# SharperJBCA/COMAPreduce

Hardware: AMD Instinct MI355X
Metric: TOD samples x channels / s (L1 -> L2 reduction) (higher is better)
Workload: dtype f32 in, f64 accumulate

## Files before the change

### comapreduce_amd/_native.py

```python
import ctypes
import os
import threading

_HERE = os.path.dirname(os.path.abspath(__file__))
LIB_PATH = os.environ.get('COMAP_HIP_LIB') or os.path.join(_HERE, '_lib', 'libcomap_hip.so')

_lib = None
_lock = threading.Lock()
_ctx = {}

c_int, c_int32, c_int64, c_double, c_void_p = ctypes.c_int, ctypes.c_int32, ctypes.c_int64, ctypes.c_double, ctypes.c_void_p
P_double = ctypes.POINTER(ctypes.c_double)
P_int32 = ctypes.POINTER(ctypes.c_int32)
P_int64 = ctypes.POINTER(ctypes.c_int64)


class ObsDesc(ctypes.Structure):
    _fields_ = [('n_feeds', c_int32), ('n_bands', c_int32), ('n_channels', c_int32),
                ('n_scans', c_int32), ('n_samples', c_int64), ('tod', c_void_p), ('el', c_void_p),
                ('n_units', c_int32), ('units_host', P_int32)]


_SIGS = {
    'comap_ctx_create': (c_int, [c_int, ctypes.POINTER(c_void_p)]),
    'comap_ctx_destroy': (c_int, [c_void_p]),
    'comap_last_error': (ctypes.c_char_p, [c_void_p]),
    'comap_set_stream': (c_int, [c_void_p, c_void_p]),
    'comap_synchronize': (c_int, [c_void_p]),
    'comap_version': (ctypes.c_char_p, []),
    'comap_host_alloc': (c_int, [ctypes.c_size_t, ctypes.POINTER(c_void_p)]),
    'comap_host_free': (None, [c_void_p]),
    'comap_cache_trim': (c_int, []),
    'comap_cache_bytes': (c_int, [P_int64, P_int64, P_int64]),
    'comap_medfilt_f64': (c_int, [c_void_p, P_double, c_int64, c_int32]),
    'comap_medfilt_batch_f64': (c_int, [c_void_p, P_double, P_int64, c_int32, c_int32, c_int32, P_double]),
    'comap_bin_values_f64': (c_int, [c_void_p, P_double, c_int64, P_int64, P_double, P_int64, c_int64]),
    'comap_l1_plan_create': (c_int, [c_void_p, ctypes.POINTER(ObsDesc), ctypes.POINTER(c_void_p)]),
    'comap_l1_plan_destroy': (c_int, [c_void_p]),
    'comap_l1_vane': (c_int, [c_void_p, c_int64, c_int64, P_int32, P_int64, P_int32, P_int64, c_double,
                              c_void_p, c_void_p]),
    'comap_l1_prefetch': (c_int, [c_void_p]),
    'comap_l1_atmosphere': (c_int, [c_void_p, P_int32, c_int32, c_void_p]),
    'comap_l1_average': (c_int, [c_void_p, c_void_p, c_void_p, c_void_p, c_int32, c_void_p, c_void_p, c_void_p]),
    'comap_l1_debug_fetch': (c_int, [c_void_p, c_int32, P_double, c_int64]),
    'comap_l1_channel_bin': (c_int, [c_void_p, c_int32, c_void_p, c_void_p, c_void_p, c_void_p, c_void_p]),
    'comap_l1_profile': (c_int, [c_void_p, c_int32]),
    'comap_l1_profile_collect': (c_int, [c_void_p, P_double, P_int64, c_int32]),
    'comap_spikes': (c_int, [c_void_p, c_void_p, c_int32, c_int64, P_int64, c_int32, c_int32, c_int32, c_double,
                             c_void_p]),
    'comap_power_spectra': (c_int, [c_void_p, c_void_p, c_int32, c_int64, P_int64, c_int32, c_void_p, c_int32,
                                    P_int64, c_void_p]),
    'comap_synth_tod': (c_int, [c_void_p, c_int32, c_int32, c_int64, ctypes.c_uint64, c_void_p, c_void_p, c_void_p,
                                c_void_p, c_void_p]),
    'comap_destripe_create': (c_int, [c_void_p, c_void_p, c_void_p, c_void_p, c_int64, c_int32, c_int64,
                                      ctypes.POINTER(c_void_p)]),
    'comap_destripe_dist_bin': (c_int, [c_void_p, c_void_p, c_void_p, c_void_p]),
    'comap_destripe_dist_parts': (c_int32, []),
    'comap_destripe_dist_project_parts': (c_int, [c_void_p, c_void_p, c_void_p, c_void_p, c_void_p, c_void_p,
                                                  c_void_p]),
    'comap_destripe_dist_update_fused': (c_int, [c_void_p, c_void_p, c_void_p, c_void_p, c_void_p, c_void_p,
                                                 c_void_p, c_void_p, c_void_p]),
    'comap_destripe_dist_direction_fused': (c_int, [c_void_p, c_void_p, c_void_p, c_void_p, c_void_p, c_void_p]),
    'comap_destripe_create_bands': (c_int, [c_void_p, c_void_p, c_void_p, c_void_p, c_void_p, c_int64, c_int32,
                                            c_int64, c_int32, ctypes.POINTER(c_void_p)]),
    'comap_destripe_create_keyed': (c_int, [c_void_p, c_void_p, c_void_p, c_void_p, c_void_p, c_void_p, c_int64,
                                            c_int64, c_int32, c_int64, c_int32, ctypes.POINTER(c_void_p)]),
    'comap_offset_centroid_keys': (c_int, [c_void_p, c_void_p, c_int64, c_int32, c_int64, c_int64, c_void_p, c_int64,
                                           c_void_p]),
    'comap_destripe_destroy': (c_int, [c_void_p]),
    'comap_destripe_n_offsets': (c_int64, [c_void_p]),
    'comap_destripe_n_bands': (c_int32, [c_void_p]),
    'comap_destripe_offsets_natural': (c_int, [c_void_p, c_void_p, c_void_p]),
    'comap_destripe_nnz': (c_int, [c_void_p, P_int64, P_int64]),
    'comap_destripe_entry_bytes': (ctypes.c_int32, [c_void_p]),
    'comap_destripe_sell_entries': (c_int64, [c_void_p]),
    'comap_destripe_local_maps': (c_int, [c_void_p, c_void_p, c_void_p, c_void_p]),
    'comap_destripe_bin': (c_int, [c_void_p, c_void_p, c_int32, c_void_p]),
    'comap_destripe_project': (c_int, [c_void_p, c_void_p, c_void_p, c_void_p, c_void_p, c_void_p]),
    'comap_destripe_dot': (c_int, [c_void_p, c_void_p, c_void_p, c_void_p]),
    'comap_destripe_cg_update': (c_int, [c_void_p, c_void_p, c_void_p, c_void_p, c_void_p, c_void_p, c_void_p,
                                         c_void_p]),
    'comap_destripe_cg_direction': (c_int, [c_void_p, c_void_p, c_void_p, c_void_p, c_void_p]),
    'comap_destripe_div_map': (c_int, [c_void_p, c_void_p, c_void_p, c_void_p]),
    'comap_relabel_pixels': (c_int, [c_void_p, c_void_p, c_int64, c_void_p, c_int64, c_int64, c_void_p]),
    'comap_relabel_pixels_tiled': (c_int, [c_void_p, c_void_p, c_int64, c_int64, c_int64, c_int32, c_void_p]),
    'comap_destripe_solve': (c_int, [c_void_p, c_double, c_int32, c_void_p, c_void_p, c_void_p, c_void_p,
                                     c_void_p, P_int32]),
    'comap_destripe_ground_create': (c_int, [c_void_p, c_void_p, c_void_p, c_void_p, c_void_p, c_void_p, c_int64,
                                             ctypes.POINTER(c_void_p)]),
    'comap_destripe_ground_destroy': (c_int, [c_void_p]),
    'comap_destripe_ground_n_groups': (c_int64, [c_void_p]),
    'comap_destripe_ground_nnz': (c_int, [c_void_p, P_int64, P_int64]),
    'comap_destripe_ground_stats': (c_int, [c_void_p, c_void_p, c_void_p]),
    'comap_destripe_ground_fold': (c_int, [c_void_p, c_void_p, c_void_p, c_void_p]),
    'comap_destripe_ground_bin': (c_int, [c_void_p, c_void_p, c_void_p]),
    'comap_destripe_ground_project': (c_int, [c_void_p, c_void_p, c_void_p, c_void_p, c_void_p, c_void_p, c_void_p]),
    'comap_destripe_ground_rhs': (c_int, [c_void_p, c_void_p, c_void_p, c_void_p, c_void_p]),
    'comap_destripe_ground_tail_dot': (c_int, [c_void_p, c_void_p, c_void_p, c_void_p]),
    'comap_destripe_ground_tail_update': (c_int, [c_void_p, c_void_p, c_void_p, c_void_p, c_void_p, c_void_p, c_void_p,
                                                  c_void_p]),
    'comap_destripe_ground_tail_direction': (c_int, [c_void_p, c_void_p, c_void_p, c_void_p, c_void_p]),
    'comap_destripe_ground_wrapped': (c_int, [c_void_p, c_void_p]),
    'comap_destripe_ground_solve': (c_int, [c_void_p, c_double, c_int32, c_void_p, c_void_p, c_void_p, c_void_p,
                                            c_void_p, P_int32]),
    'comap_destripe_ground_dist_bin': (c_int, [c_void_p, c_void_p, c_void_p, c_void_p]),
    'comap_destripe_ground_dist_project': (c_int, [c_void_p, c_void_p, c_void_p, c_void_p, c_void_p, c_void_p,
                                                   c_void_p]),
    'comap_destripe_ground_dist_update': (c_int, [c_void_p, c_void_p, c_void_p, c_void_p, c_void_p, c_void_p,
                                                  c_void_p]),
    'comap_destripe_ground_dist_direction': (c_int, [c_void_p, c_void_p, c_void_p, c_void_p, c_void_p]),
    'comap_destripe_prior_create': (c_int, [c_void_p, c_void_p, c_int64, c_void_p, c_int32, ctypes.POINTER(c_void_p)]),
    'comap_destripe_prior_destroy': (c_int, [c_void_p]),
    'comap_destripe_prior_tile': (c_int32, []),
    'comap_destripe_prior_apply': (c_int, [c_void_p, c_void_p, c_void_p, c_int32]),
    'comap_destripe_prior_apply_dot': (c_int, [c_void_p, c_void_p, c_void_p, c_int32, c_void_p]),
    'comap_destripe_prior_solve': (c_int, [c_void_p, c_double, c_int32, c_void_p, c_void_p, c_void_p, c_void_p,
                                           c_void_p, P_int32]),
    'comap_destripe_mask_view': (c_int, [c_void_p, c_void_p, c_void_p, c_void_p, c_void_p, ctypes.POINTER(c_void_p)]),
    'comap_destripe_solve_view': (c_int, [c_void_p, c_double, c_int32, c_void_p, c_void_p, c_void_p, c_void_p,
                                          c_void_p, P_int32]),
    'comap_destripe_split_maps': (c_int, [c_void_p, c_void_p, c_void_p, c_void_p, c_void_p, c_void_p, c_void_p, c_int32,
                                          c_int64, c_int32, c_int64, c_int32, c_void_p, c_void_p, c_void_p, c_void_p]),
    'comap_destripe_split_div': (c_int, [c_void_p, c_void_p, c_void_p, c_void_p, c_int64, c_void_p, c_void_p]),
# ... 149 lines not shown
```

### comapreduce_amd/csrc/l1_kernels.hip

```cpp
#include "comap_internal.h"

#include <algorithm>
#include <cfloat>
#include <cmath>
#include <cstdlib>
#include <cstring>
#include <type_traits>
#include <utility>

using namespace comap;

#ifndef COMAP_GROUPS
#define COMAP_GROUPS 0
#endif
constexpr int kGroupsAutoMin = 3;

typedef float f32x4u __attribute__((ext_vector_type(4), aligned(4)));
__device__ __forceinline__ f32x4u ld4(const float *p)
{
    return __builtin_nontemporal_load(reinterpret_cast<const f32x4u *>(p));
}

__device__ __forceinline__ double wave_sum(double v)
{
// ... 218 lines not shown
        const int f = units[4 * u], t0 = units[4 * u + 2], n = units[4 * u + 3];
        const int t = blockIdx.x * blockDim.x + threadIdx.x;
        if (t >= n) continue;
        const float *p = tod + (int64_t)(f * kBands + b) * kChannels * T + t0 + t;
        bool ok = true;
        for (int c = 10; c < 1014; ++c)
            if (atmos_channel(c) && !isfinite(p[(int64_t)c * T])) ok = false;
        valid[voff[pr] + t] = ok;
    }
}

__global__ void __launch_bounds__(256) k_masked_fit_sums(const float *__restrict__ tod, const double *__restrict__ A,
                                                         const int32_t *__restrict__ units,
                                                         const int32_t *__restrict__ pairs, int64_t T,
                                                         const int64_t *__restrict__ voff,
                                                         const uint8_t *__restrict__ valid, int64_t UC,
                                                         double *__restrict__ fs, double *__restrict__ ub,
                                                         const int32_t *__restrict__ list,
                                                         const int32_t *__restrict__ count)
{
    const int np = *count;
    for (int li = blockIdx.y; li < np; li += gridDim.y) {
    const int pr = list[li];
    const int u = pairs[2 * pr], b = pairs[2 * pr + 1];
    const int f = units[4 * u], t0 = units[4 * u + 2], n = units[4 * u + 3];
    const int wid = threadIdx.x >> 6, lane = threadIdx.x & 63;
    const int c = blockIdx.x * 4 + wid;
    const float *p = tod + ((int64_t)(f * kBands + b) * kChannels + c) * T + t0;
    const double *a = A + (int64_t)f * T + t0;
    const uint8_t *v = valid + voff[pr];
    double s0 = 0, s1 = 0, cn = 0, sa = 0, saa = 0;
    for (int t = lane; t < n; t += 64) {
        if (!v[t]) continue;
        const double x = p[t], at = a[t];
        s0 += x;
        s1 = fma(at, x, s1);
        cn += 1.0;
        sa += at;
        saa = fma(at, at, saa);
    }
    s0 = wave_sum(s0); s1 = wave_sum(s1);
    cn = wave_sum(cn); sa = wave_sum(sa); saa = wave_sum(saa);
    if (lane == 0) {
        const int64_t i = (int64_t)u * kBC + b * kChannels + c;
        fs[i] = s0;
        fs[UC + i] = s1;
        if (c == 0) {
            double *o = ub + 4 * ((int64_t)u * kBands + b);
            o[0] = cn; o[1] = sa; o[2] = saa;
        }
    }
    }
}

__global__ void __launch_bounds__(256) k_pair_flags(const int32_t *__restrict__ rowbad, int npairs,
                                                    int32_t *__restrict__ flag)
{
    const int lane = threadIdx.x & 63;
    const int pr = blockIdx.x * 4 + (threadIdx.x >> 6);
    if (pr >= npairs) return;
    const int u = pr / kBands, b = pr % kBands;
    const int32_t *rb = rowbad + (int64_t)u * kBC + b * kChannels;
    bool any = false;
    for (int c = lane; c < kChannels; c += 64) any |= atmos_channel(c) && rb[c] > 0;
    any = __ballot(any) != 0ull;
    if (lane == 0) flag[pr] = any ? 1 : 0;
}

__global__ void k_pair_list(const int32_t *__restrict__ flag, int npairs, int32_t *__restrict__ list,
                            int32_t *__restrict__ count)
{
    const int lane = threadIdx.x & 63;
    int base = 0;
    for (int i0 = 0; i0 < npairs; i0 += 64) {
        const int i = i0 + lane;
        const bool f = i < npairs && flag[i];
        const unsigned long long m = __ballot(f);
        if (f) list[base + __popcll(m & ((1ull << lane) - 1ull))] = i;
        base += __popcll(m);
    }
    if (lane == 0) *count = base;
}

__global__ void k_ub_from_units(const double *__restrict__ us, int U, double *__restrict__ ub)
{
    const int i = blockIdx.x * blockDim.x + threadIdx.x;
    if (i >= U * kBands) return;
    const double *q = us + 8 * (int64_t)(i / kBands);
    ub[4 * (int64_t)i] = q[0];
    ub[4 * (int64_t)i + 1] = q[1];
    ub[4 * (int64_t)i + 2] = q[2];
}

__global__ void __launch_bounds__(256) k_fill_rows(float *__restrict__ tod, const int64_t *__restrict__ rows,
                                                   const float *__restrict__ med, int nrows, int64_t *__restrict__ pos,
                                                   int64_t cap, int64_t *__restrict__ npos)
{
    const int r = blockIdx.y;
    if (r >= nrows) return;
    const int64_t off = rows[2 * r];
    float *p = tod + off;
    const int64_t n = rows[2 * r + 1];
    const float m = med[r];
    for (int64_t i = blockIdx.x * (int64_t)blockDim.x + threadIdx.x; i < n; i += (int64_t)gridDim.x * blockDim.x)
        if (isnan(p[i])) {
            const unsigned long long k = atomicAdd(reinterpret_cast<unsigned long long *>(npos), 1ull);
            if ((int64_t)k < cap) {
                pos[k] = off + i;
                p[i] = m;
            }
        }
}

__global__ void k_restore_nan(float *__restrict__ tod, const int64_t *__restrict__ pos, const int64_t *__restrict__ npos,
                              int64_t cap)
{
    const int64_t n = min(*npos, cap);
    for (int64_t i = blockIdx.x * (int64_t)blockDim.x + threadIdx.x; i < n; i += (int64_t)gridDim.x * blockDim.x)
        tod[pos[i]] = __int_as_float(0x7fc00000);
}

__global__ void k_fit_from_median(const int32_t *__restrict__ units, const int32_t *__restrict__ ulist, int nu,
                                  const float *__restrict__ med, int F, double *__restrict__ fit)
{
    const int64_t i = blockIdx.x * (int64_t)blockDim.x + threadIdx.x;
    if (i >= (int64_t)nu * kBC) return;
    const int k = (int)(i / kBC), bc = (int)(i % kBC);
    const int u = ulist[k];
    const int f = units[4 * u], s = units[4 * u + 1];
    const int b = bc / kChannels, c = bc % kChannels;
    double *o = fit + (((int64_t)s * F + f) * kBands + b) * 2 * kChannels;
    o[c] = (double)med[i];
    o[kChannels + c] = 0.0;
}

__global__ void k_atmos_fit(const int32_t *__restrict__ units, const double *__restrict__ ubs,
                            const double *__restrict__ fs, int64_t UC, int F, int U,
                            double *__restrict__ fit, const double *__restrict__ fs_sel = nullptr,
                            const int32_t *__restrict__ sel = nullptr)
{
    const int64_t i = blockIdx.x * (int64_t)blockDim.x + threadIdx.x;
    if (i >= (int64_t)U * kBC) return;
    const int u = (int)(i / kBC);
    const int bc = (int)(i % kBC);
    const int b = bc / kChannels, c = bc % kChannels;
    const int f = units[4 * u], s = units[4 * u + 1];
    const double *q = ubs + 4 * ((int64_t)u * kBands + b);
    const double n = q[0], sa = q[1], saa = q[2];
    double o = NAN, a = NAN;
    if (atmos_channel(c) && n >= 100.0) {
        const double *src = (sel && sel[(int64_t)u * kBands + b]) ? fs_sel : fs;
        const double sd = src[i], sad = src[UC + i];
        const double det = n * saa - sa * sa;
        o = (saa * sd - sa * sad) / det;
        a = (n * sad - sa * sd) / det;
    }
    double *out = fit + (((int64_t)s * F + f) * kBands + b) * 2 * kChannels;
    out[c] = o;
    out[kChannels + c] = a;
}

__global__ void __launch_bounds__(256) k_coef_b(const int32_t *__restrict__ units, const double *__restrict__ us,
                                                const double *__restrict__ mom, int64_t UC,
                                                const double *__restrict__ fit, int F, const float *__restrict__ med,
                                                double *__restrict__ oa,
                                                double *__restrict__ alpha, double *__restrict__ nf,
                                                double *__restrict__ bsum, int32_t *__restrict__ flag)
{
    __shared__ double red[4];
    const int ub = blockIdx.x;
    const int u = ub / kBands, b = ub % kBands;
    const int n = units[4 * u + 3];
    if (ub == 0 && threadIdx.x < comap_l1_plan::kMaxGroups) flag[threadIdx.x] = 0;
    const int fu = units[4 * u], su = units[4 * u + 1];
    const double *fo = fit + (((int64_t)su * F + fu) * kBands + b) * 2 * kChannels;
    const double *q = us + 8 * (int64_t)u;
    const double sv = q[3], svv = q[4], n4 = q[5];
    double beta = 0, gamma = 0, cnt = 0;
    for (int c = threadIdx.x; c < kChannels; c += blockDim.x) {
        const int64_t i = (int64_t)u * kBC + b * kChannels + c;
        const double o = med ? (double)med[i] : fo[c], a = med ? 0.0 : fo[kChannels + c];
        oa[2 * i] = o;
        oa[2 * i + 1] = a;
        double rms = NAN;
        if (n4 > 0 && isfinite(o) && isfinite(a)) {
            const double su = mom[2 * UC + i], suu = mom[3 * UC + i], suv = mom[4 * UC + i];
            const double mean = (su - a * sv) / n4;
            double var = (suu - 2.0 * a * suv + a * a * svv) / n4 - mean * mean;
            var = var < 0.0 ? 0.0 : var;
            rms = sqrt(var) / sqrt(2.0) * sqrt(kDnuTau);
        }
        nf[i] = rms;
        double al = 0.0;
        if (median_channel(c)) {
            al = 1.0 / rms;
            if (isfinite(al) && isfinite(o) && isfinite(a)) {
                beta += al * o;
                gamma += al * a;
                cnt += 1.0;
            } else {
                al = 0.0;
            }
        }
        alpha[i] = al;
    }
    beta = block_sum256(beta, red);
    gamma = block_sum256(gamma, red);
    cnt = block_sum256(cnt, red);
    if (threadIdx.x == 0) {
        double *o = bsum + 4 * (int64_t)ub;
        o[0] = beta; o[1] = gamma; o[2] = cnt;
        o[3] = (cnt > 0 && n >= 2 * kMedfiltWindow) ? 1.0 : 0.0;
    }
}


constexpr int kJ = kTile / 256;
template <int J = kJ>
__device__ __forceinline__ void load_groups(const float *__restrict__ p, int nv0, double (&x)[4 * J])
{
#pragma unroll
    for (int g = 0; g < J; ++g) {
        const int nv = nv0 - 256 * g;
        if (nv >= 4) {
            const f32x4u v = *reinterpret_cast<const f32x4u *>(p + 256 * g);
            x[4 * g] = v.x; x[4 * g + 1] = v.y; x[4 * g + 2] = v.z; x[4 * g + 3] = v.w;
        } else {
#pragma unroll
            for (int e = 0; e < 4; ++e) x[4 * g + e] = (e < nv) ? (double)p[256 * g + e] : 0.0;
        }
    }
}

template <int J, bool FULL>
// ... 679 lines not shown
{
    const int np = n / 2;
    double s = 0, cnt = 0;
    for (int k = threadIdx.x; k < np; k += blockDim.x) {
        const double d = r[2 * k + 1] - r[2 * k];
        if (!isnan(d)) { s += d; cnt += 1.0; }
    }
    s = block_sum256(s, red);
    cnt = block_sum256(cnt, red);
    const double mean = s / cnt;
    double v = 0;
    for (int k = threadIdx.x; k < np; k += blockDim.x) {
        const double d = r[2 * k + 1] - r[2 * k];
        if (!isnan(d)) v += (d - mean) * (d - mean);
    }
    v = block_sum256(v, red);
    const double rms = sqrt(v / cnt) / sqrt(2.0);
    const double wt = 1.0 / (rms * rms);
    for (int t = threadIdx.x; t < n; t += blockDim.x) wo[t] = wt;
}

__global__ void __launch_bounds__(256) k_scan_weights(int ub0, const int32_t *__restrict__ units, int64_t T,
                                                      const double *__restrict__ tod_out, double *__restrict__ w_out)
{
    __shared__ double red[4];
    const int ub = ub0 + blockIdx.x;
    const int u = ub / kBands, b = ub % kBands;
    const int f = units[4 * u], t0 = units[4 * u + 2], n = units[4 * u + 3];
    const int64_t o = (int64_t)(f * kBands + b) * T + t0;
    scan_weight_band(tod_out + o, n, w_out + o, red);
}

__global__ void __launch_bounds__(256) k_finish(const int32_t *__restrict__ units, const int32_t *__restrict__ tiles,
                                                int64_t tile0, int64_t T, const double *__restrict__ A,
                                                const double *__restrict__ mf, const double *__restrict__ dsum,
                                                double *__restrict__ tod_out, double *__restrict__ orig_out,
                                                double *__restrict__ dG, const int32_t *__restrict__ flag)
{
    if (*flag != 0) return;
    const int64_t tile = tile0 + blockIdx.x;
    const int u = tiles[2 * tile];
    const int f = units[4 * u], t0 = units[4 * u + 2], n = units[4 * u + 3];
    const double *ds = dsum + 16 * (int64_t)u * kBands;
    for (int k = threadIdx.x; k < kTile; k += 256) {
        const int r = tiles[2 * tile + 1] + k;
        if (r >= n) break;
        const int64_t t = t0 + r;
        const double a = A[(int64_t)f * T + t];
        double m[kBands], g = dG[(int64_t)f * T + t];
#pragma unroll
        for (int b = 0; b < kBands; ++b) {
            m[b] = mf[(int64_t)(f * kBands + b) * T + t];
            const double *d = ds + 16 * b;
            g += d[0] + a * d[1] + m[b] * d[2];
        }
        dG[(int64_t)f * T + t] = g;
#pragma unroll
        for (int b = 0; b < kBands; ++b) {
            const double *d = ds + 16 * b;
            const int64_t o = (int64_t)(f * kBands + b) * T + t;
            tod_out[o] = (tod_out[o] + d[3] + a * d[4] + m[b] * d[5] - g * d[9]) / d[10];
            orig_out[o] = (orig_out[o] + d[6] + a * d[7] + m[b] * d[8]) / d[11];
        }
    }
}

__global__ void __launch_bounds__(256) k_zero_gaps(const int64_t *__restrict__ gaps, int64_t T, int F,
                                                   double *__restrict__ tod_out, double *__restrict__ orig_out,
                                                   double *__restrict__ w_out)
{
    const int64_t *g = gaps + 3 * (int64_t)blockIdx.y;
    const int64_t f = g[0], t0 = g[1], n = g[2];
    for (int64_t k = blockIdx.x * (int64_t)blockDim.x + threadIdx.x; k < n; k += (int64_t)gridDim.x * blockDim.x) {
#pragma unroll
        for (int b = 0; b < kBands; ++b) {
            const int64_t o = (f * kBands + b) * T + t0 + k;
            tod_out[o] = 0.0;
            orig_out[o] = 0.0;
            w_out[o] = 0.0;
        }
    }
}

__global__ void __launch_bounds__(256) k_vane(const float *__restrict__ tod, int64_t T, int F,
                                              int64_t vstart, const int32_t *__restrict__ hot,
                                              const int64_t *__restrict__ hoff, const int32_t *__restrict__ cold,
                                              const int64_t *__restrict__ coff, double t_hot,
                                              double *__restrict__ tsys, double *__restrict__ gain)
{
    __shared__ float s_cold[128];
    const int side = threadIdx.x >> 7;
    const int64_t row = (int64_t)blockIdx.x * 128 + (threadIdx.x & 127);
    const bool live = row < (int64_t)F * kBC;
    const int fb = live ? (int)(row / kChannels) : 0;
    const float *p = tod + row * T + vstart;
    const int64_t h0 = hoff[fb], h1 = hoff[fb + 1], k0 = coff[fb], k1 = coff[fb + 1];
    float mean = 0.f;
    if (live && h1 != h0) {
        const int32_t *idx = side == 0 ? hot : cold;
        const int64_t j0 = side == 0 ? h0 : k0, j1 = side == 0 ? h1 : k1;
        float s = 0.f;
        int64_t cnt = 0;
        constexpr int kV = 16;
        int64_t j = j0;
        for (; j + kV <= j1; j += kV) {
            float x[kV];
#pragma unroll
            for (int k = 0; k < kV; ++k) x[k] = p[idx[j + k]];
#pragma unroll
            for (int k = 0; k < kV; ++k) {
                const bool ok = !isnan(x[k]);
                s += ok ? x[k] : 0.f;
                cnt += ok;
            }
        }
        for (; j < j1; ++j) {
            const float x = p[idx[j]];
            const bool ok = !isnan(x);
            s += ok ? x : 0.f;
            cnt += ok;
        }
        mean = (float)((double)s / (double)cnt);
    }
    if (side == 1) s_cold[threadIdx.x & 127] = mean;
    __syncthreads();
    if (side == 1 || !live) return;
    if (h1 == h0) {
        gain[row] = 0.0;
        tsys[row] = 0.0;
        return;
    }
    const float mc = s_cold[threadIdx.x];
    const float d = mean - mc;
    const double g = (double)d / (t_hot - 2.73);
    gain[row] = g;
    tsys[row] = (double)mc / g;
}

__global__ void __launch_bounds__(256) k_channel_bin(const float *__restrict__ tod, int64_t T, int32_t bw,
                                                     int32_t nbin, const double *__restrict__ w,
                                                     const double *__restrict__ g, const double *__restrict__ wsum,
                                                     double *__restrict__ avg, double *__restrict__ sd)
{
#pragma clang fp contract(off)
    const int b = uniform(threadIdx.x >> 6);
    const int lane = threadIdx.x & 63;
    const int64_t ntile = (T + kTile - 1) / kTile;
    const int f = (int)(blockIdx.x / ntile);
    const int64_t t0 = (int64_t)(blockIdx.x % ntile) * kTile;
    const int64_t r0 = t0 + 4 * lane;
    const int nv0 = (int)std::max<int64_t>(-1, std::min<int64_t>(T - r0, 1 << 20));
    const int64_t fb = (int64_t)f * kBands + b;
    const float *base = tod + fb * kChannels * T + r0;
    const double *wc = w + fb * kChannels, *gc = g + fb * kChannels;
    const bool full = t0 + kTile <= T;
    for (int k = 0; k < nbin; ++k) {
        double s1[4 * kJ], s2[4 * kJ];
#pragma unroll
        for (int i = 0; i < 4 * kJ; ++i) s1[i] = s2[i] = 0.0;
        for (int c = k * bw; c < (k + 1) * bw; ++c) {
            const double wv = wc[c], gv = gc[c];
            f32x4u r[kJ];
            if (full) load_raw<kJ, true>(base + (int64_t)c * T, nv0, r);
            else load_raw<kJ, false>(base + (int64_t)c * T, nv0, r);
#pragma unroll
            for (int q = 0; q < kJ; ++q)
#pragma unroll
                for (int e = 0; e < 4; ++e) {
                    const float x = (float)((double)r[q][e] / gv);
                    s1[4 * q + e] += (double)x * wv;
                    s2[4 * q + e] += (double)(x * x) * wv;
                }
        }
        const double W = wsum[fb * nbin + k];
        double *ao = avg + (fb * nbin + k) * T + r0, *so = sd + (fb * nbin + k) * T + r0;
#pragma unroll
        for (int q = 0; q < kJ; ++q)
#pragma unroll
            for (int e = 0; e < 4; ++e) {
                const int o = 256 * q + e;
                if (o >= nv0) continue;
                const double a = s1[4 * q + e] / W, sq = s2[4 * q + e] / W;
                ao[o] = a;
                so[o] = sqrt(sq - a * a);
            }
    }
}

static int prof_begin(comap_l1_plan *p, int id, hipStream_t st)
{
    if (!p->prof_on) return -1;
    if (p->prof_level == 1 && id != KV_MOMENTS && id != KV_BAND_SUMS && id != KV_REGRESS) return -1;
    const int idx = (int)p->prof_rec.size() * 2;
    while ((int)p->prof_pool.size() < idx + 2) {
        hipEvent_t e;
        if (hipEventCreate(&e) != hipSuccess) return -1;
        p->prof_pool.push_back(e);
    }
    (void)hipEventRecord(p->prof_pool[idx], st);
    return idx;
}

static void prof_end(comap_l1_plan *p, int id, int idx, hipStream_t st)
{
    if (idx < 0) return;
    (void)hipEventRecord(p->prof_pool[idx + 1], st);
    p->prof_rec.push_back({id, idx});
}

#define PROF_ON(p, id, st, ...)              \
    do {                                     \
        const int _pi = prof_begin(p, id, st); \
        __VA_ARGS__;                         \
        prof_end(p, id, _pi, st);            \
    } while (0)
#define PROF(p, id, ...) PROF_ON(p, id, (p)->ctx->stream, __VA_ARGS__)

extern "C" int comap_l1_profile(comap_l1_plan *p, int32_t enable)
{
// ... 228 lines not shown
    for (hipEvent_t e : p->prof_pool) (void)hipEventDestroy(e);
    delete p;
    return 0;
}

static int launch_moments(comap_l1_plan *p)
{
    comap_ctx *ctx = p->ctx;
    const int64_t UC = (int64_t)p->U * kBC;
    if (!p->pre_a_ev) COMAP_CHECK(ctx, hipEventCreateWithFlags(&p->pre_a_ev, hipEventDisableTiming));
    COMAP_CHECK(ctx, hipEventRecord(p->pre_a_ev, ctx->stream));
    p->pre_a_valid = true;
    COMAP_CHECK(ctx, hipMemsetAsync(p->nan_count, 0, 4, ctx->stream));
    const int64_t grid = (int64_t)p->U * kBands * (kChannels / (4 * kCPW));
    PROF(p, KV_MOMENTS, k_moments<<<grid, 256, 0, ctx->stream>>>(p->tod, p->airmass, p->units, p->T, p->mom, UC,
                                                                     p->nan_count, p->rowbad));
    COMAP_LAUNCH_CHECK(ctx);
    COMAP_CHECK(ctx, hipMemcpyAsync(p->nan_host, p->nan_count, 4, hipMemcpyDeviceToHost, ctx->stream));
    COMAP_CHECK(ctx, hipEventRecord(p->mom_event, ctx->stream));
    p->moments_pending = true;
    p->moments_valid = true;
    return 0;
}

static int wait_moments(comap_l1_plan *p)
{
    if (!p->moments_pending) return 0;
    COMAP_CHECK(p->ctx, hipEventSynchronize(p->mom_event));
    p->nan_total = *p->nan_host;
    p->moments_pending = false;
    return 0;
}

static int run_moments(comap_l1_plan *p)
{
    int rc = launch_moments(p);
    return rc ? rc : wait_moments(p);
}

extern "C" int comap_l1_prefetch(comap_l1_plan *p)
{
    if (!p) return -1;
    COMAP_DEVICE_GUARD(p->ctx);
    int rc = launch_moments(p);
    if (!rc) p->prefetched = true;
    return rc;
}

static int fetch_rowbad(comap_l1_plan *p, std::vector<int32_t> &rb)
{
    comap_ctx *ctx = p->ctx;
    rb.resize((size_t)p->U * kBC);
    COMAP_CHECK(ctx, hipMemcpyAsync(rb.data(), p->rowbad, 4 * rb.size(), hipMemcpyDeviceToHost, ctx->stream));
    COMAP_CHECK(ctx, hipStreamSynchronize(ctx->stream));
    return 0;
}

static int unit_row_medians(comap_l1_plan *p, const std::vector<int64_t> &rowids, float *med_dev)
{
    std::vector<int64_t> rows(2 * rowids.size());
    for (size_t k = 0; k < rowids.size(); ++k) {
        const int64_t i = rowids[k];
        const int u = (int)(i / kBC), bc = (int)(i % kBC);
        const int32_t *q = &p->units_h[4 * u];
        rows[2 * k] = ((int64_t)q[0] * kBC + bc) * p->T + q[2];
        rows[2 * k + 1] = q[3];
    }
    return comap_row_nanmedian(p->ctx, p->tod, rows.data(), (int32_t)rowids.size(), med_dev);
}

extern "C" int comap_l1_atmosphere(comap_l1_plan *p, const int32_t *const_el_units, int32_t n_const_el,
                                   double *fit)
{
    if (!p || !fit) return -1;
    COMAP_DEVICE_GUARD(p->ctx);
    p->pre_a_valid = false;
    comap_ctx *ctx = p->ctx;
    hipStream_t st = ctx->stream;
    int rc = p->prefetched ? 0 : launch_moments(p);
    p->prefetched = false;
    if (rc) return rc;
    const int64_t UC = (int64_t)p->U * kBC;
    const int UB = p->U * kBands;
    k_ub_from_units<<<(UB + 255) / 256, 256, 0, st>>>(p->unit_sums, p->U, p->ubs);
    COMAP_LAUNCH_CHECK(ctx);
    if (!p->sel_pairs) {
        std::vector<int32_t> pairs(2 * (size_t)UB);
        std::vector<int64_t> voff(UB + 1, 0);
        int maxn = 0;
        for (int u = 0; u < p->U; ++u)
            for (int b = 0; b < kBands; ++b) {
                const int pr = u * kBands + b;
                pairs[2 * pr] = u;
                pairs[2 * pr + 1] = b;
                voff[pr + 1] = voff[pr] + p->units_h[4 * u + 3];
                maxn = std::max(maxn, p->units_h[4 * u + 3]);
            }
        COMAP_CHECK(ctx, hipMalloc((void **)&p->sel_pairs, 4 * pairs.size()));
        COMAP_CHECK(ctx, hipMalloc((void **)&p->sel_voff, 8 * voff.size()));
        COMAP_CHECK(ctx, hipMalloc((void **)&p->sel_flag, 4 * (2 * (size_t)UB + 1)));
        COMAP_CHECK(ctx, hipMalloc((void **)&p->sel_valid, (size_t)voff.back() + 1));
        COMAP_CHECK(ctx, comap_upload(p->sel_pairs, pairs.data(), 4 * pairs.size(), st));
        COMAP_CHECK(ctx, comap_upload(p->sel_voff, voff.data(), 8 * voff.size(), st));
        p->sel_maxn = maxn;
    }
    int32_t *plist = p->sel_flag + UB, *pcount = p->sel_flag + 2 * UB;
    k_pair_flags<<<(UB + 3) / 4, 256, 0, st>>>(p->rowbad, UB, p->sel_flag);
    COMAP_LAUNCH_CHECK(ctx);
    k_pair_list<<<1, 64, 0, st>>>(p->sel_flag, UB, plist, pcount);
    COMAP_LAUNCH_CHECK(ctx);
    if (p->sel_maxn > 0) {
        const unsigned gy = (unsigned)std::min(UB, 16);
        k_select_time<<<dim3((p->sel_maxn + 255) / 256, gy), 256, 0, st>>>(p->tod, p->units, p->sel_pairs, p->T,
                                                                           p->sel_voff, p->sel_valid, plist, pcount);
        COMAP_LAUNCH_CHECK(ctx);
        k_masked_fit_sums<<<dim3(kChannels / 4, gy), 256, 0, st>>>(p->tod, p->airmass, p->units, p->sel_pairs, p->T,
                                                                   p->sel_voff, p->sel_valid, UC, p->fitsum, p->ubs,
                                                                   plist, pcount);
        COMAP_LAUNCH_CHECK(ctx);
    }
    const double *fs = p->mom;
    PROF(p, KV_ATMOS_FIT, k_atmos_fit<<<(UC + 255) / 256, 256, 0, st>>>(p->units, p->ubs, fs, UC, p->F, p->U, fit,
                                                                        p->fitsum, p->sel_flag));
    COMAP_LAUNCH_CHECK(ctx);
    if (n_const_el > 0) {
        std::vector<int64_t> ids;
        for (int k = 0; k < n_const_el; ++k) {
            const int u = const_el_units[k];
            if (u < 0 || u >= p->U) return comap_fail(ctx, -1, "constant-elevation unit out of range");
            for (int bc = 0; bc < kBC; ++bc) ids.push_back((int64_t)u * kBC + bc);
        }
        float *med = nullptr;
        int32_t *dl = nullptr;
        DevTemps tmp(st);
        COMAP_CHECK(ctx, tmp.alloc(&med, ids.size()));
        COMAP_CHECK(ctx, tmp.alloc(&dl, (size_t)n_const_el));
        COMAP_CHECK(ctx, hipMemcpyAsync(dl, const_el_units, 4 * (size_t)n_const_el, hipMemcpyHostToDevice, st));
        if ((rc = unit_row_medians(p, ids, med))) return rc;
        const int64_t nt = (int64_t)n_const_el * kBC;
        k_fit_from_median<<<(nt + 255) / 256, 256, 0, st>>>(p->units, dl, n_const_el, med, p->F, fit);
        COMAP_LAUNCH_CHECK(ctx);
    }
    return 0;
}

static int fill_nan_rows(comap_l1_plan *p)
{
    comap_ctx *ctx = p->ctx;
    hipStream_t st = ctx->stream;
    std::vector<int32_t> rb;
    int rc = fetch_rowbad(p, rb);
    if (rc) return rc;
    std::vector<int64_t> ids;
    for (size_t i = 0; i < rb.size(); ++i)
        if (rb[i] > 0) ids.push_back((int64_t)i);
    if (ids.empty()) return 0;
    float *med = nullptr;
    int64_t *drows = nullptr;
    std::vector<int64_t> rows(2 * ids.size());
    for (size_t k = 0; k < ids.size(); ++k) {
        const int u = (int)(ids[k] / kBC), bc = (int)(ids[k] % kBC);
        const int32_t *q = &p->units_h[4 * u];
        rows[2 * k] = ((int64_t)q[0] * kBC + bc) * p->T + q[2];
        rows[2 * k + 1] = q[3];
    }
    DevTemps tmp(st);
    COMAP_CHECK(ctx, tmp.alloc(&med, ids.size()));
    COMAP_CHECK(ctx, tmp.alloc(&drows, rows.size()));
    const int64_t cap = std::max<int64_t>(p->nan_total, 1);
    if (cap > p->nanpos_cap) {
        if (p->nanpos) (void)hipFree(p->nanpos);
        p->nanpos = nullptr;
        p->nanpos_cap = 0;
        COMAP_CHECK(ctx, hipMalloc((void **)&p->nanpos, 8 * (size_t)cap));
        p->nanpos_cap = cap;
    }
    if (!p->nanpos_n) COMAP_CHECK(ctx, hipMalloc((void **)&p->nanpos_n, 8));
    COMAP_CHECK(ctx, hipMemsetAsync(p->nanpos_n, 0, 8, st));
    COMAP_CHECK(ctx, hipMemcpyAsync(drows, rows.data(), 8 * rows.size(), hipMemcpyHostToDevice, st));
    if ((rc = comap_row_nanmedian(ctx, p->tod, rows.data(), (int32_t)ids.size(), med))) return rc;
    p->filled = true;
    for (size_t r0 = 0; r0 < ids.size(); r0 += 65535) {
        const int nr = (int)std::min<size_t>(65535, ids.size() - r0);
        k_fill_rows<<<dim3(16, nr), 256, 0, st>>>(const_cast<float *>(p->tod), drows + 2 * r0, med + r0, nr,
                                                  p->nanpos, p->nanpos_cap, p->nanpos_n);
        COMAP_LAUNCH_CHECK(ctx);
    }
    return run_moments(p);
}

static int restore_nan(comap_l1_plan *p)
{
    if (!p->filled) return 0;
    comap_ctx *ctx = p->ctx;
    k_restore_nan<<<256, 256, 0, ctx->stream>>>(const_cast<float *>(p->tod), p->nanpos, p->nanpos_n, p->nanpos_cap);
    p->filled = false;
    p->moments_valid = false;
    COMAP_LAUNCH_CHECK(ctx);
    return 0;
}

extern "C" int comap_l1_average(comap_l1_plan *p, const double *fit, const double *tsys0, const double *gain0,
                                int32_t calibrator, double *tod_out, double *orig_out, double *w_out)
{
    if (!p || !fit || !tsys0 || !gain0 || !tod_out || !orig_out || !w_out) return -1;
    COMAP_DEVICE_GUARD(p->ctx);
// ... 124 lines not shown
    }
    const int gs = (G > 1 && !special) ? G - 1 : G;
    for (int g = 0; g < gs; ++g)
        if (side != st) COMAP_CHECK(ctx, hipStreamWaitEvent(st, p->ev_m[g], 0));
    if ((rc = regress(0, gs, st))) return rc;
    if (!special && (rc = tail(0, gs, st))) return rc;
    if (gs < G) {
        COMAP_CHECK(ctx, hipStreamWaitEvent(st, p->ev_m[G - 1], 0));
        if ((rc = regress(G - 1, G, st))) return rc;
        if ((rc = tail(G - 1, G, st))) return rc;
    }
    side_join.armed = false;
    if (!special) return 0;
    PROF(p, KV_COEF_D, coef_d(1, 0, UB, p->flag, nullptr, st));
    COMAP_LAUNCH_CHECK(ctx);
    COMAP_CHECK(ctx, hipMemsetAsync(p->ugate, 0, 4 * (size_t)p->U, st));
    special_rows(0);
    COMAP_LAUNCH_CHECK(ctx);
    coef_d(2, 0, UB, p->flag, p->ugate, st);
    COMAP_LAUNCH_CHECK(ctx);
    COMAP_CHECK(ctx, hipMemsetAsync(p->flag, 0xff, 4, st));
    PROF(p, KV_GAIN_AVG, k_gain_avg<<<p->n_tiles, 256, 0, st>>>(p->tod, p->airmass, p->units, p->tiles, 0, p->T, UC,
                                                                p->kap, p->dsum, p->mf, tod_out, orig_out, p->dG,
                                                                p->flag));
    COMAP_LAUNCH_CHECK(ctx);
    PROF(p, KV_FINISH, k_finish<<<p->n_tiles, 256, 0, st>>>(p->units, p->tiles, 0, p->T, p->airmass, p->mf, p->dsum,
                                                            tod_out, orig_out, p->dG, p->flag));
    COMAP_LAUNCH_CHECK(ctx);
    special_rows(1);
    COMAP_LAUNCH_CHECK(ctx);
    PROF(p, KV_SCAN_WEIGHTS, k_scan_weights<<<UB, 256, 0, st>>>(0, p->units, p->T, tod_out, w_out));
    COMAP_LAUNCH_CHECK(ctx);
    return 0;
}


extern "C" int comap_l1_vane(comap_l1_plan *p, int64_t vstart, int64_t vlen, const int32_t *hot_h,
                             const int64_t *hoff_h, const int32_t *cold_h, const int64_t *coff_h,
                             double t_hot, double *tsys, double *gain)
{
    if (!p || !hoff_h || !coff_h || !tsys || !gain) return -1;
    COMAP_DEVICE_GUARD(p->ctx);
    comap_ctx *ctx = p->ctx;
    const int FB = p->F * kBands;
    if (vstart < 0 || vstart + vlen > p->T) return comap_fail(ctx, -1, "vane event out of range");
    const int64_t nh = hoff_h[FB], nc = coff_h[FB];
    for (int64_t i = 0; i < nh; ++i)
        if (hot_h[i] < 0 || hot_h[i] >= vlen) return comap_fail(ctx, -1, "hot index out of range");
    for (int64_t i = 0; i < nc; ++i)
        if (cold_h[i] < 0 || cold_h[i] >= vlen) return comap_fail(ctx, -1, "cold index out of range");
    const size_t off_c = (size_t)nh * 4, off_ho = (off_c + (size_t)nc * 4 + 15) & ~(size_t)15;
    const size_t off_co = off_ho + (size_t)(FB + 1) * 8, bytes = off_co + (size_t)(FB + 1) * 8;
    hipStream_t st = ctx->stream;
    static const bool use_side = getenv("COMAP_VANE_SIDE") && getenv("COMAP_VANE_SIDE")[0] == '1';
    hipStream_t vs = (use_side && p->side) ? p->side : st;
    if (vs != st) {
        if (!p->pre_a_ev) COMAP_CHECK(ctx, hipEventCreateWithFlags(&p->pre_a_ev, hipEventDisableTiming));
        if (!p->vane_done) COMAP_CHECK(ctx, hipEventCreateWithFlags(&p->vane_done, hipEventDisableTiming));
        if (!p->pre_a_valid) COMAP_CHECK(ctx, hipEventRecord(p->pre_a_ev, st));
        COMAP_CHECK(ctx, hipStreamWaitEvent(vs, p->pre_a_ev, 0));
    }
    if (!p->vane_ev) COMAP_CHECK(ctx, hipEventCreateWithFlags(&p->vane_ev, hipEventDisableTiming));
    else COMAP_CHECK(ctx, hipEventSynchronize(p->vane_ev));
    if (bytes > p->vane_cap) {
        if (p->vane_pinned) (void)hipHostFree(p->vane_pinned);
        if (p->vane_dev) (void)hipFree(p->vane_dev);
        p->vane_pinned = p->vane_dev = nullptr;
        p->vane_cap = 0;
        COMAP_CHECK(ctx, hipHostMalloc((void **)&p->vane_pinned, bytes, hipHostMallocDefault));
        COMAP_CHECK(ctx, hipMalloc((void **)&p->vane_dev, bytes));
        p->vane_cap = bytes;
    }
    std::memcpy(p->vane_pinned, hot_h, (size_t)nh * 4);
    std::memcpy(p->vane_pinned + off_c, cold_h, (size_t)nc * 4);
    std::memcpy(p->vane_pinned + off_ho, hoff_h, (size_t)(FB + 1) * 8);
    std::memcpy(p->vane_pinned + off_co, coff_h, (size_t)(FB + 1) * 8);
    COMAP_CHECK(ctx, hipMemcpyAsync(p->vane_dev, p->vane_pinned, bytes, hipMemcpyHostToDevice, vs));
    COMAP_CHECK(ctx, hipEventRecord(p->vane_ev, vs));
    const int32_t *dh = (const int32_t *)p->vane_dev;
    const int32_t *dc = (const int32_t *)(p->vane_dev + off_c);
    const int64_t *dho = (const int64_t *)(p->vane_dev + off_ho);
    const int64_t *dco = (const int64_t *)(p->vane_dev + off_co);
    const int64_t rows = (int64_t)FB * kChannels;
    PROF_ON(p, KV_VANE, vs, k_vane<<<(rows + 127) / 128, 256, 0, vs>>>(p->tod, p->T, p->F, vstart, dh, dho, dc, dco,
                                                                      t_hot, tsys, gain));
    COMAP_LAUNCH_CHECK(ctx);
    if (vs != st) {
        COMAP_CHECK(ctx, hipEventRecord(p->vane_done, vs));
        COMAP_CHECK(ctx, hipStreamWaitEvent(st, p->vane_done, 0));
    }
    return 0;
}

extern "C" int comap_l1_debug_fetch(comap_l1_plan *p, int32_t what, double *out, int64_t n)
{
    if (!p || !out) return -1;
    COMAP_DEVICE_GUARD(p->ctx);
    comap_ctx *ctx = p->ctx;
    const int64_t UC = (int64_t)p->U * kBC;
    const double *src = nullptr;
    int64_t cnt = 0;
    switch (what) {
    case 0: src = p->nf; cnt = UC; break;
    case 1: src = p->mf; cnt = (int64_t)p->F * kBands * p->T; break;
    case 2: src = p->dG; cnt = (int64_t)p->F * p->T; break;
    case 3: src = p->xreg; cnt = 2 * UC; break;
    case 4: src = p->mb; cnt = (int64_t)p->F * kBands * p->T; break;
    case 5: src = p->kap; cnt = 3 * UC; break;
    case 6: src = p->dsum; cnt = (int64_t)p->U * kBands * 16; break;
    case 7: src = p->alpha; cnt = UC; break;
    case 8: src = p->oa; cnt = 2 * UC; break;
    case 10: {
        const int UB = p->U * kBands;
        if (n < (int64_t)UB) return comap_fail(ctx, -1, "debug buffer too small");
        std::vector<int32_t> c(UB);
        COMAP_CHECK(ctx, hipMemcpyAsync(c.data(), p->needc, 4 * (size_t)UB, hipMemcpyDeviceToHost, ctx->stream));
        COMAP_CHECK(ctx, hipStreamSynchronize(ctx->stream));
        for (int i = 0; i < UB; ++i) out[i] = c[i];
        return 0;
    }
    case 9: {
        const int UB = p->U * kBands;
        if (n < 2 * (int64_t)UB) return comap_fail(ctx, -1, "debug buffer too small");
        std::vector<int32_t> c(UB);
        std::vector<double> bs(4 * (size_t)UB);
        COMAP_CHECK(ctx, hipMemcpyAsync(c.data(), p->dcnt, 4 * (size_t)UB, hipMemcpyDeviceToHost, ctx->stream));
        COMAP_CHECK(ctx, hipMemcpyAsync(bs.data(), p->bsum, 32 * (size_t)UB, hipMemcpyDeviceToHost, ctx->stream));
        COMAP_CHECK(ctx, hipStreamSynchronize(ctx->stream));
        for (int i = 0; i < UB; ++i) { out[2 * i] = c[i]; out[2 * i + 1] = bs[4 * (size_t)i + 3] > 0 ? 1.0 : 0.0; }
        return 0;
    }
    default: return comap_fail(ctx, -1, "unknown debug array");
    }
    if (n < cnt) return comap_fail(ctx, -1, "debug buffer too small");
    COMAP_CHECK(ctx, hipMemcpyAsync(out, src, cnt * 8, hipMemcpyDeviceToHost, ctx->stream));
    COMAP_CHECK(ctx, hipStreamSynchronize(ctx->stream));
    return 0;
}

extern "C" int comap_l1_channel_bin(comap_l1_plan *p, int32_t bin_size, const double *weights, const double *gain,
                                    const double *wsum, double *avg, double *stddev)
{
    if (!p || !weights || !gain || !wsum || !avg || !stddev) return -1;
    COMAP_DEVICE_GUARD(p->ctx);
    p->pre_a_valid = false;
    comap_ctx *ctx = p->ctx;
    if (bin_size < 1 || kChannels % bin_size) return comap_fail(ctx, -1, "bin_size must divide 1024");
    const int64_t ntile = (p->T + kTile - 1) / kTile;
    k_channel_bin<<<(unsigned)(p->F * ntile), 256, 0, ctx->stream>>>(p->tod, p->T, bin_size, kChannels / bin_size,
                                                                     weights, gain, wsum, avg, stddev);
    COMAP_LAUNCH_CHECK(ctx);
    return 0;
}
```

### include/comap_hip.h

```cpp
#ifndef COMAP_HIP_H
#define COMAP_HIP_H

#include <stdint.h>

#ifdef __cplusplus
extern "C" {
#endif

typedef struct comap_ctx comap_ctx;
typedef struct comap_l1_plan comap_l1_plan;
typedef struct comap_destriper comap_destriper;

int comap_ctx_create(int device, comap_ctx **out);
int comap_ctx_destroy(comap_ctx *ctx);
const char *comap_last_error(const comap_ctx *ctx);
int comap_set_stream(comap_ctx *ctx, void *stream);
int comap_synchronize(comap_ctx *ctx);
const char *comap_version(void);
int comap_host_alloc(size_t bytes, void **out);
void comap_host_free(void *p);
int comap_cache_trim(void);
int comap_cache_bytes(int64_t *device_cached, int64_t *device_live, int64_t *host_cached);

int comap_medfilt_f64(comap_ctx *ctx, double *x_host, int64_t n, int32_t w);
int comap_medfilt_batch_f64(comap_ctx *ctx, const double *x_host, const int64_t *offsets_host,
                            int32_t nseries, int32_t w, int32_t mode, double *out_host);
int comap_bin_values_f64(comap_ctx *ctx, double *image_host, int64_t npix,
                         const int64_t *pixels_host, const double *weights_host,
                         const int64_t *mask_host, int64_t n);

typedef struct {
    int32_t n_feeds;
    int32_t n_bands;
    int32_t n_channels;
    int32_t n_scans;
    int64_t n_samples;
    const float *tod;
    const double *el;
    int32_t n_units;
    const int32_t *units_host;
} comap_obs_desc;

int comap_l1_plan_create(comap_ctx *ctx, const comap_obs_desc *desc, comap_l1_plan **out);
int comap_l1_plan_destroy(comap_l1_plan *plan);

int comap_l1_vane(comap_l1_plan *plan, int64_t vane_start, int64_t vane_len,
                  const int32_t *hot_idx_host, const int64_t *hot_off_host,
                  const int32_t *cold_idx_host, const int64_t *cold_off_host,
                  double t_hot, double *tsys_dev, double *gain_dev);

int comap_l1_prefetch(comap_l1_plan *plan);
int comap_l1_atmosphere(comap_l1_plan *plan, const int32_t *const_el_units_host, int32_t n_const_el,
                        double *fit_values_dev);

int comap_l1_average(comap_l1_plan *plan, const double *fit_values_dev,
                     const double *tsys0_dev, const double *gain0_dev, int32_t calibrator,
                     double *tod_out_dev, double *orig_out_dev, double *weights_out_dev);

int comap_l1_channel_bin(comap_l1_plan *plan, int32_t bin_size, const double *weights_dev,
                         const double *gain_dev, const double *wsum_dev, double *avg_dev, double *stddev_dev);

int comap_l1_debug_fetch(comap_l1_plan *plan, int32_t what, double *out_host, int64_t n);

int comap_l1_profile(comap_l1_plan *plan, int32_t enable);
int comap_l1_profile_collect(comap_l1_plan *plan, double *ms_host, int64_t *counts_host, int32_t n);

int comap_spikes(comap_ctx *ctx, const double *tod_dev, int32_t n_rows, int64_t n_samples,
                 const int64_t *edges_host, int32_t n_scans, int32_t medfilt_window, int32_t step,
                 double threshold, uint8_t *mask_dev);

int comap_power_spectra(comap_ctx *ctx, const double *tod_dev, int32_t n_rows, int64_t n_samples,
                        const int64_t *edges_host, int32_t n_scans, const uint8_t *mask_dev, int32_t mode,
                        const int64_t *out_offsets_host, double *out_dev);

int comap_synth_tod(comap_ctx *ctx, int32_t n_feeds, int32_t feed0, int64_t n_samples, uint64_t seed,
                    const double *level_dev, const double *mult_dev, const double *hot_dev,
                    float *tod_dev, float *band_average_dev);

int comap_destripe_create(comap_ctx *ctx, const int32_t *pixels_dev, const double *tod_dev,
                          const double *weights_dev, int64_t n_samples, int32_t offset_length,
                          int64_t npix, comap_destriper **out);
int comap_destripe_create_bands(comap_ctx *ctx, const int32_t *pixels_dev, const double *tod_dev,
                                const double *weights_dev, const uint8_t *keep_dev, int64_t n_samples,
                                int32_t offset_length, int64_t npix, int32_t n_bands, comap_destriper **out);
int comap_destripe_create_keyed(comap_ctx *ctx, const int32_t *pixels_dev, const double *tod_dev,
                                const double *weights_dev, const uint8_t *keep_dev, const int32_t *okey_dev,
                                int64_t okey_max, int64_t n_samples, int32_t offset_length, int64_t npix,
                                int32_t n_bands, comap_destriper **out);
int comap_destripe_destroy(comap_destriper *d);
int64_t comap_destripe_n_offsets(const comap_destriper *d);
int32_t comap_destripe_n_bands(const comap_destriper *d);
int comap_destripe_offsets_natural(comap_destriper *d, const double *x_internal_dev, double *x_out_dev);
int comap_destripe_nnz(const comap_destriper *d, int64_t *nnz_offset_major, int64_t *nnz_pixel_major);
int32_t comap_destripe_entry_bytes(const comap_destriper *d);
int64_t comap_destripe_sell_entries(const comap_destriper *d);
int comap_destripe_local_maps(comap_destriper *d, double *h_dev, double *hits_dev, double *naive_num_dev);
int comap_destripe_bin(comap_destriper *d, const double *x_dev, int32_t mode, double *num_dev);
int comap_destripe_project(comap_destriper *d, const double *x_dev, const double *num_dev,
                           const double *h_dev, double *y_dev, double *dot_dev);
int comap_destripe_dot(comap_destriper *d, const double *a_dev, const double *b_dev, double *dot_dev);
int comap_destripe_cg_update(comap_destriper *d, const double *rr_dev, const double *pq_dev,
                             double *x_dev, double *r_dev, const double *p_dev, const double *q_dev,
                             double *rr_new_dev);
int comap_destripe_cg_direction(comap_destriper *d, const double *rr_new_dev, const double *rr_dev,
                                double *p_dev, const double *r_dev);
int comap_destripe_dist_bin(comap_destriper *d, const double *p_dev, double *num_dev, const int32_t *flags_dev);
int32_t comap_destripe_dist_parts(void);
int comap_destripe_dist_project_parts(comap_destriper *d, const double *p_dev, const double *num_dev,
                                      const double *h_dev, double *q_dev, double *pq_part_dev,
                                      const int32_t *flags_dev);
int comap_destripe_dist_update_fused(comap_destriper *d, double *scal_dev, const double *pq_part_dev, double *x_dev,
                                     double *r_dev, const double *p_dev, const double *q_dev, double *rr_part_dev,
                                     const int32_t *flags_dev);
int comap_destripe_dist_direction_fused(comap_destriper *d, double *scal_dev, const double *rr_part_dev,
                                        double *p_dev, const double *r_dev, int32_t *flags_dev);
int comap_destripe_div_map(comap_destriper *d, const double *num_dev, const double *h_dev, double *out_dev);
int comap_destripe_solve(comap_destriper *d, double threshold, int32_t niter, double *x_dev,
                         double *map_dev, double *naive_dev, double *weight_dev,
                         double *hits_dev, int32_t *iters_out);
int comap_relabel_pixels_tiled(comap_ctx *ctx, const int32_t *pix_dev, int64_t n, int64_t nx, int64_t ny, int32_t T,
                               int32_t *out_dev);
int comap_offset_centroid_keys(comap_ctx *ctx, const int32_t *pix_dev, int64_t n, int32_t offset_length, int64_t nx,
                               int64_t ny, const int32_t *lut_dev, int64_t n_internal, int32_t *key_dev);
int comap_relabel_pixels(comap_ctx *ctx, const int32_t *pix_dev, int64_t n, const int32_t *lut_dev, int64_t npix,
                         int64_t n_internal, int32_t *out_dev);

typedef struct comap_ground comap_ground;
int comap_destripe_ground_create(comap_destriper *d, const int32_t *pixels_dev, const double *az_dev,
                                 const double *tod_dev, const double *weights_dev, const int32_t *gid_dev,
                                 int64_t n_groups, comap_ground **out);
int comap_destripe_ground_destroy(comap_ground *g);
int64_t comap_destripe_ground_n_groups(const comap_ground *g);
// ... 108 lines not shown
```

Before: 766.5 billion.

## Restructure vane kernel to gather samples cooperatively via LDS tiles

Rewrites the vane hot/cold mean kernel so that 64-row blocks within one feed-band gather chunks of 32 indexed samples. Lanes map to samples, so the loads along a row are coalesced, and the values are staged through a double-sided LDS tile. The next chunk is prefetched while the current one is reduced. Separately, it removes the k_ub_from_units launch by having k_atmos_fit read unit sums directly when a band is not selected. This adds __syncthreads per chunk, and the k_vane grid now assumes the row count is a multiple of 64.

```diff
diff --git a/comapreduce_amd/_native.py b/comapreduce_amd/_native.py
--- a/comapreduce_amd/_native.py
+++ b/comapreduce_amd/_native.py
@@ -39,6 +39,7 @@
     'comap_l1_plan_destroy': (c_int, [c_void_p]),
     'comap_l1_vane': (c_int, [c_void_p, c_int64, c_int64, P_int32, P_int64, P_int32, P_int64, c_double,
                               c_void_p, c_void_p]),
+    'comap_l1_vane_chunk': (c_int32, []),
     'comap_l1_prefetch': (c_int, [c_void_p]),
     'comap_l1_atmosphere': (c_int, [c_void_p, P_int32, c_int32, c_void_p]),
     'comap_l1_average': (c_int, [c_void_p, c_void_p, c_void_p, c_void_p, c_int32, c_void_p, c_void_p, c_void_p]),
diff --git a/comapreduce_amd/csrc/l1_kernels.hip b/comapreduce_amd/csrc/l1_kernels.hip
--- a/comapreduce_amd/csrc/l1_kernels.hip
+++ b/comapreduce_amd/csrc/l1_kernels.hip
@@ -324,16 +324,6 @@
     if (lane == 0) *count = base;
 }
 
-__global__ void k_ub_from_units(const double *__restrict__ us, int U, double *__restrict__ ub)
-{
-    const int i = blockIdx.x * blockDim.x + threadIdx.x;
-    if (i >= U * kBands) return;
-    const double *q = us + 8 * (int64_t)(i / kBands);
-    ub[4 * (int64_t)i] = q[0];
-    ub[4 * (int64_t)i + 1] = q[1];
-    ub[4 * (int64_t)i + 2] = q[2];
-}
-
 __global__ void __launch_bounds__(256) k_fill_rows(float *__restrict__ tod, const int64_t *__restrict__ rows,
                                                    const float *__restrict__ med, int nrows, int64_t *__restrict__ pos,
                                                    int64_t cap, int64_t *__restrict__ npos)
@@ -377,7 +367,7 @@
 }
 
 __global__ void k_atmos_fit(const int32_t *__restrict__ units, const double *__restrict__ ubs,
-                            const double *__restrict__ fs, int64_t UC, int F, int U,
+                            const double *__restrict__ us, const double *__restrict__ fs, int64_t UC, int F, int U,
                             double *__restrict__ fit, const double *__restrict__ fs_sel = nullptr,
                             const int32_t *__restrict__ sel = nullptr)
 {
@@ -387,11 +377,12 @@
     const int bc = (int)(i % kBC);
     const int b = bc / kChannels, c = bc % kChannels;
     const int f = units[4 * u], s = units[4 * u + 1];
-    const double *q = ubs + 4 * ((int64_t)u * kBands + b);
+    const bool picked = sel && sel[(int64_t)u * kBands + b];
+    const double *q = picked ? ubs + 4 * ((int64_t)u * kBands + b) : us + 8 * (int64_t)u;
     const double n = q[0], sa = q[1], saa = q[2];
     double o = NAN, a = NAN;
     if (atmos_channel(c) && n >= 100.0) {
-        const double *src = (sel && sel[(int64_t)u * kBands + b]) ? fs_sel : fs;
+        const double *src = picked ? fs_sel : fs;
         const double sd = src[i], sad = src[UC + i];
         const double det = n * saa - sa * sa;
         o = (saa * sd - sa * sad) / det;
@@ -1237,59 +1228,102 @@
     }
 }
 
+constexpr int kVaneRows = 64;
+constexpr int kVaneChunk = 32;
+constexpr int kVaneStride = kVaneChunk + 1;
+static_assert(kChannels % kVaneRows == 0, "a vane block stays inside one (feed, band)");
+
 __global__ void __launch_bounds__(256) k_vane(const float *__restrict__ tod, int64_t T, int F,
                                               int64_t vstart, const int32_t *__restrict__ hot,
                                               const int64_t *__restrict__ hoff, const int32_t *__restrict__ cold,
                                               const int64_t *__restrict__ coff, double t_hot,
                                               double *__restrict__ tsys, double *__restrict__ gain)
 {
-    __shared__ float s_cold[128];
-    const int side = threadIdx.x >> 7;
-    const int64_t row = (int64_t)blockIdx.x * 128 + (threadIdx.x & 127);
-    const bool live = row < (int64_t)F * kBC;
-    const int fb = live ? (int)(row / kChannels) : 0;
-    const float *p = tod + row * T + vstart;
-    const int64_t h0 = hoff[fb], h1 = hoff[fb + 1], k0 = coff[fb], k1 = coff[fb + 1];
-    float mean = 0.f;
-    if (live && h1 != h0) {
-        const int32_t *idx = side == 0 ? hot : cold;
-        const int64_t j0 = side == 0 ? h0 : k0, j1 = side == 0 ? h1 : k1;
-        float s = 0.f;
-        int64_t cnt = 0;
-        constexpr int kV = 16;
-        int64_t j = j0;
-        for (; j + kV <= j1; j += kV) {
-            float x[kV];
-#pragma unroll
-            for (int k = 0; k < kV; ++k) x[k] = p[idx[j + k]];
-#pragma unroll
-            for (int k = 0; k < kV; ++k) {
-                const bool ok = !isnan(x[k]);
-                s += ok ? x[k] : 0.f;
-                cnt += ok;
+    __shared__ float tile[2][kVaneRows * kVaneStride];
+    __shared__ float s_cold[kVaneRows];
+    const int fb = uniform((int)(blockIdx.x / (kChannels / kVaneRows)));
+    const int64_t row0 = (int64_t)blockIdx.x * kVaneRows;
+    const int64_t h0 = hoff[fb], k0 = coff[fb];
+    const int nh = (int)(hoff[fb + 1] - h0), nk = (int)(coff[fb + 1] - k0);
+    if (nh == 0) {
+        if (threadIdx.x < kVaneRows) {
+            gain[row0 + threadIdx.x] = 0.0;
+            tsys[row0 + threadIdx.x] = 0.0;
+        }
+        return;
+    }
+    const int wave = uniform(threadIdx.x >> 6), lane = threadIdx.x & 63;
+    const int smp = lane & (kVaneChunk - 1);
+    const int lrow = wave * 16 + (lane >> 5);
+    const float *base = tod + (row0 + lrow) * T + vstart;
+    const int nchunk = (std::max(nh, nk) + kVaneChunk - 1) / kVaneChunk;
+    float xh[8] = {}, xc[8] = {};
+    int ih = 0, ic = 0;
+    auto load_idx = [&](int c) {
+        const int j = c * kVaneChunk + smp;
+        if (c * kVaneChunk < nh) ih = hot[h0 + std::min(j, nh - 1)];
+        if (c * kVaneChunk < nk) ic = cold[k0 + std::min(j, nk - 1)];
+    };
+    auto load_smp = [&](int c) {
+        const bool dh = c * kVaneChunk < nh, dc = c * kVaneChunk < nk;
+        if (dh) {
+#pragma unroll
+            for (int i = 0; i < 8; ++i) xh[i] = base[(int64_t)(2 * i) * T + ih];
+        }
+        if (dc) {
+#pragma unroll
+            for (int i = 0; i < 8; ++i) xc[i] = base[(int64_t)(2 * i) * T + ic];
+        }
+    };
+    load_idx(0);
+    load_smp(0);
+    load_idx(1);
+    const int side = wave;
+    const int nlist = side == 0 ? nh : nk;
+    float s = 0.f;
+    int cnt = 0;
+    for (int c = 0; c < nchunk; ++c) {
+#pragma unroll
+        for (int i = 0; i < 8; ++i) {
+            tile[0][(lrow + 2 * i) * kVaneStride + smp] = xh[i];
+            tile[1][(lrow + 2 * i) * kVaneStride + smp] = xc[i];
+        }
+        __syncthreads();
+        if (c + 1 < nchunk) {
+            load_smp(c + 1);
+            load_idx(c + 2);
+        }
+        if (side < 2) {
+            const float *tl = &tile[side][lane * kVaneStride];
+            const int n = nlist - c * kVaneChunk;
+            if (n >= kVaneChunk) {
+#pragma unroll
+                for (int k = 0; k < kVaneChunk; ++k) {
+                    const float x = tl[k];
+                    const bool ok = !isnan(x);
+                    s += ok ? x : 0.f;
+                    cnt += ok;
+                }
+            } else {
+                for (int k = 0; k < n; ++k) {
+                    const float x = tl[k];
+                    const bool ok = !isnan(x);
+                    s += ok ? x : 0.f;
+                    cnt += ok;
+                }
             }
         }
-        for (; j < j1; ++j) {
-            const float x = p[idx[j]];
-            const bool ok = !isnan(x);
-            s += ok ? x : 0.f;
-            cnt += ok;
-        }
-        mean = (float)((double)s / (double)cnt);
-    }
-    if (side == 1) s_cold[threadIdx.x & 127] = mean;
+        __syncthreads();
+    }
+    const float mean = (float)((double)s / (double)cnt);
+    if (side == 1) s_cold[lane] = mean;
     __syncthreads();
-    if (side == 1 || !live) return;
-    if (h1 == h0) {
-        gain[row] = 0.0;
-        tsys[row] = 0.0;
-        return;
-    }
-    const float mc = s_cold[threadIdx.x];
+    if (side != 0) return;
+    const float mc = s_cold[lane];
     const float d = mean - mc;
     const double g = (double)d / (t_hot - 2.73);
-    gain[row] = g;
-    tsys[row] = (double)mc / g;
+    gain[row0 + lane] = g;
+    tsys[row0 + lane] = (double)mc / g;
 }
 
 __global__ void __launch_bounds__(256) k_channel_bin(const float *__restrict__ tod, int64_t T, int32_t bw,
@@ -1684,8 +1718,6 @@
     if (rc) return rc;
     const int64_t UC = (int64_t)p->U * kBC;
     const int UB = p->U * kBands;
-    k_ub_from_units<<<(UB + 255) / 256, 256, 0, st>>>(p->unit_sums, p->U, p->ubs);
-    COMAP_LAUNCH_CHECK(ctx);
     if (!p->sel_pairs) {
         std::vector<int32_t> pairs(2 * (size_t)UB);
         std::vector<int64_t> voff(UB + 1, 0);
@@ -1722,8 +1754,10 @@
         COMAP_LAUNCH_CHECK(ctx);
     }
     const double *fs = p->mom;
-    PROF(p, KV_ATMOS_FIT, k_atmos_fit<<<(UC + 255) / 256, 256, 0, st>>>(p->units, p->ubs, fs, UC, p->F, p->U, fit,
-                                                                        p->fitsum, p->sel_flag));
+    PROF(p, KV_ATMOS_FIT, k_atmos_fit<<<(UC + 255) / 256, 256, 0, st>>>(p->units, p->ubs, p->unit_sums, fs,
+                                                                        UC, p->F, p->U, fit,
+                                                                        p->fitsum,
+                                                                        p->sel_maxn > 0 ? p->sel_flag : nullptr));
     COMAP_LAUNCH_CHECK(ctx);
     if (n_const_el > 0) {
         std::vector<int64_t> ids;
@@ -2014,7 +2048,7 @@
     const int64_t *dho = (const int64_t *)(p->vane_dev + off_ho);
     const int64_t *dco = (const int64_t *)(p->vane_dev + off_co);
     const int64_t rows = (int64_t)FB * kChannels;
-    PROF_ON(p, KV_VANE, vs, k_vane<<<(rows + 127) / 128, 256, 0, vs>>>(p->tod, p->T, p->F, vstart, dh, dho, dc, dco,
+    PROF_ON(p, KV_VANE, vs, k_vane<<<rows / kVaneRows, 256, 0, vs>>>(p->tod, p->T, p->F, vstart, dh, dho, dc, dco,
                                                                       t_hot, tsys, gain));
     COMAP_LAUNCH_CHECK(ctx);
     if (vs != st) {
@@ -2023,6 +2057,8 @@
     }
     return 0;
 }
+
+extern "C" int32_t comap_l1_vane_chunk(void) { return kVaneChunk; }
 
 extern "C" int comap_l1_debug_fetch(comap_l1_plan *p, int32_t what, double *out, int64_t n)
 {
diff --git a/include/comap_hip.h b/include/comap_hip.h
--- a/include/comap_hip.h
+++ b/include/comap_hip.h
@@ -48,6 +48,7 @@
                   const int32_t *hot_idx_host, const int64_t *hot_off_host,
                   const int32_t *cold_idx_host, const int64_t *cold_off_host,
                   double t_hot, double *tsys_dev, double *gain_dev);
+int32_t comap_l1_vane_chunk(void);
 
 int comap_l1_prefetch(comap_l1_plan *plan);
 int comap_l1_atmosphere(comap_l1_plan *plan, const int32_t *const_el_units_host, int32_t n_const_el,
```

Result: no change. 773.0 billion, median of 6 (+0.8%).
